# sanweiliti/RoHM

Hardware: AMD Instinct MI355X
Metric: denoised 145-frame clips/sec @1000 DDPM steps (higher is better)
Workload: dtype f32

## Files before the change

rohm_amd/csrc/common.h:

```cpp
#pragma once
#include <hip/hip_runtime.h>
#include <stdint.h>
#include <stdio.h>
#include <stdarg.h>
#include "../../include/rohm_hip.h"

typedef float f32x4 __attribute__((ext_vector_type(4)));
typedef float f32x2 __attribute__((ext_vector_type(2)));

namespace rohm {

void set_error(const char* fmt, ...);

#define ROHM_HIP_CHECK(expr)                                                             \
    do {                                                                                 \
        hipError_t _e = (expr);                                                          \
        if (_e != hipSuccess) {                                                          \
            rohm::set_error("%s failed: %s (%s:%d)", #expr, hipGetErrorString(_e), __FILE__, \
                            __LINE__);                                                   \
            return ROHM_ERR_HIP;                                                         \
        }                                                                                \
    } while (0)

#define ROHM_LAUNCH_CHECK()                                                              \
// ... 91 lines not shown
int exchange_layout_state(int device, const char** why);
int device_of_pointer(const void* ptr);

int launch_gemm(const GemmParams& p, int epi, hipStream_t s);

struct ChainParams {
    const float* ctx; float* h; float* y; float* ff; float* qkv;
    int M, D, F, tiles_m;
    const float *out_w, *out_b, *n1_w, *n1_b, *l1_w, *l1_b, *l2_w, *l2_b, *n2_w, *n2_b, *in_w, *in_b;
    float qscale, ln_eps;
    float* xln_stats; unsigned* xln_err; const unsigned* xln_pass; unsigned* xln_xcc; unsigned epoch;
    unsigned long long* flags;
    int fault;
};
struct StackLayerW { const float *out_w, *out_b, *n1_w, *n1_b, *l1_w, *l1_b, *l2_w, *l2_b, *n2_w, *n2_b, *in_w, *in_b; };
struct StackParams {
    float *h, *y, *ff, *qkv, *ctx;
    int M, D, F, tiles_m, L, n_head;
    float qscale, ln_eps;
    float* xln_stats; unsigned* xln_err; const unsigned* xln_pass; unsigned* xln_xcc; unsigned epoch;
    unsigned long long* flags;
    int fault;
    StackLayerW layer[8];
    const float* apack; int lda_pack; const float* w_embed; int ldw_embed; int k_embed;
    int S; const float* tab; const float* tab0; int ldtab, ldtab0, tab_by_row;
    const float* w_fold; int ldw_fold; const float* qtab; const float* qtab0;
    unsigned long long* timeline;
    int tail;
    const float* t_out_w; const float* t_out_b;
    float* t_x; const float* t_cond; const float* t_noise;
    float* t_x0; float* t_apack;
    float t_c1, t_c2, t_sigma;
    int t_traj, t_C, t_T, t_lda;
    unsigned* t_pass_ctr;
    unsigned pass_add;
};
constexpr int kStackTimelineLayers = 9, kStackTimelineStamps = 12;
int launch_encoder_stack(const StackParams& p, hipStream_t s);
int encoder_chain_parts(int M, int D, int F);
bool encoder_chain_pays(int B);
size_t encoder_chain_flag_bytes(int M);
int launch_encoder_chain(const ChainParams& p, hipStream_t s);
bool stream_is_capturing(hipStream_t s);
#ifdef __HIPCC__
__device__ __forceinline__ float wave_sum64(float v) {
    typedef unsigned rohm_u2 __attribute__((ext_vector_type(2)));
    rohm_u2 s = __builtin_amdgcn_permlane32_swap(__float_as_uint(v), __float_as_uint(v), false, false);
    v = __uint_as_float(s[0]) + __uint_as_float(s[1]);
    s = __builtin_amdgcn_permlane16_swap(__float_as_uint(v), __float_as_uint(v), false, false);
    v = __uint_as_float(s[0]) + __uint_as_float(s[1]);
// ... 31 lines not shown
```

rohm_amd/csrc/encoder_chain.hip:

```cpp
#include <type_traits>
#include "common.h"
#include "gemm_sched.h"
#include "attention_tile.h"

namespace rohm {

typedef float f32x16c __attribute__((ext_vector_type(16)));

namespace chain {

constexpr int BM = 144, BK = kGemmBK, NRB = BM / 16;
constexpr int A_UNITS = BM * 8, A_ITERS = (A_UNITS + 255) / 256;
constexpr int kMaxBN = 384;
constexpr int kZone = 2 * (BM + kMaxBN) * BK;
constexpr int kLdsFloats = kZone + 512 + 4 * BM * 2;
constexpr int kSc1 = 16;

struct PhaseArgs {
    const float* A; int lda;
    const float* W; int ldw;
    float* C; int ldc;
    int K;
    const float* bias;
    const float* R; int ldr;
// ... 42 lines not shown
            if ((it & 127) == 127 && __hip_atomic_load(err, __ATOMIC_RELAXED, __HIP_MEMORY_SCOPE_AGENT) != 0u) break;
            if (it > (1 << 19)) {
                __hip_atomic_store(err, 1u, __ATOMIC_RELAXED, __HIP_MEMORY_SCOPE_AGENT);
                break;
            }
        }
    }
    __syncthreads();
}

template <int BN, int EPI, bool PREF, bool SC1, bool REFETCH, bool HEAD = false, bool FOLD = false, typename AfterLoop>
__device__ __forceinline__ void gemm_phase(const PhaseArgs& p, float* smem, const int tid, AfterLoop&& after_loop,
                                           AtQFrags<2>* q_out = nullptr) {
    static_assert(EPI == EPI_BIAS_RES_LN || EPI == EPI_BIAS_GELU || EPI == EPI_QKV || EPI == EPI_EMBED, "chain phases: LN tail, GELU, QKV, embed");
    static_assert(!HEAD || (EPI == EPI_QKV && BN == 3 * AT_DH), "the head-aligned tile is one head's q | k | v");
    static_assert(!FOLD || (EPI == EPI_QKV && PREF && !SC1), "the folded in-projection: prefetched weights, A from an earlier launch");
    constexpr int WN = BN / 4;
    constexpr int NCB = WN / 16;
    constexpr int B_ITERS = BN * 8 / 256;
    constexpr int PIECES = A_ITERS + B_ITERS;
    constexpr int AUX = SC1 ? kSc1 : 0;

    float* As = smem;
    float* Bs = smem + 2 * BM * BK;
    float* lds_dummy = smem + kZone;
    float* const zone = lds_dummy + 512;
    float* const colrow = HEAD ? smem + 2 * AT_TILE : zone;
    static_assert(!HEAD || 2 * AT_TILE + 512 <= AT_LDS_FLOATS, "head-aligned tile: the bias row overruns the stack's LDS");

    const int lane = tid & 63;
    const int wave = tid >> 6;
// ... 346 lines not shown
#pragma unroll
                for (int q = 0; q < 4; ++q) v[q] = gelu_erf(v[q]);
            }
            if constexpr (EPI == EPI_QKV) {
                if (nb < p.qcols) {
#pragma unroll
                    for (int q = 0; q < 4; ++q) v[q] *= p.qscale;
                }
            }
            *reinterpret_cast<f32x4*>(p.C + (size_t)m * p.ldc + nb) = v;
        });
    }
}

template <int G>
__device__ __forceinline__ void head_tail_phase(const StackParams& p, const int g, const int tn, float* smem, const int tid) {
    constexpr int NC_OWN = 16 / G;
    constexpr int NW = NC_OWN * 16 + 16;
    constexpr int NRMAX = (G == 4) ? 9 : 5;
    constexpr int W_UNITS = NW * 8, W_ITERS = (W_UNITS + 255) / 256;
    constexpr int PIECES = A_ITERS + W_ITERS;
    constexpr int kBuf = (BM + NW) * BK;
    static_assert(3 * kBuf <= kZone, "head phase: staging buffers overrun the zone");
    float* lds_dummy = smem + kZone;
    const int lane = tid & 63, li = lane & 15, lg = lane >> 4;
    const int wave = __builtin_amdgcn_readfirstlane(tid >> 6);
    const int wave_u = wave * 64;
    const int D = p.D, m0 = g * BM;
    int c_loc, r0, nr, e;
    if constexpr (G == 4) { c_loc = wave; r0 = 0; nr = 9; e = tn * 4 + wave; }
    else { c_loc = wave >> 1; r0 = (wave & 1) ? 5 : 0; nr = (wave & 1) ? 4 : 5; e = (wave & 1) ? tn * 2 + (wave >> 1) : 99; }
// ... 33 lines not shown
            __builtin_amdgcn_global_load_lds((const __attribute__((address_space(1))) void*)(w_src[i] + k0),
                                             (__attribute__((address_space(3))) void*)dst, 16, 0, 0);
        }
    };

    f32x4 acc[NRMAX], acc_e = f32x4{0.f, 0.f, 0.f, 0.f};
#pragma unroll
    for (int r = 0; r < NRMAX; ++r) acc[r] = f32x4{0.f, 0.f, 0.f, 0.f};
    const int nk = D / BK;
    dma(0, 0);
    dma(1, BK);

    typedef float f32x4u __attribute__((ext_vector_type(4), aligned(4)));
    const int C = p.t_C, T = p.t_T, traj = p.t_traj, S = BM;
    float* const x = p.t_x;
    const float* const nzp = p.t_noise;
    const size_t row_own = ((size_t)g * C + traj + (tn * NC_OWN + c_loc) * 16 + li) * T;
    const size_t row_sh = ((size_t)g * C + traj + 256 + li) * T;
    f32x4 xt[NRMAX], nz[NRMAX], xt_e = f32x4{0.f, 0.f, 0.f, 0.f}, nz_e = f32x4{0.f, 0.f, 0.f, 0.f};
#pragma unroll
    for (int r = 0; r < NRMAX; ++r) {
        xt[r] = nz[r] = f32x4{0.f, 0.f, 0.f, 0.f};
        if (r < nr) {
            const size_t idx = row_own + (size_t)((r0 + r) * 16 + 4 * lg) - 1;
            xt[r] = *reinterpret_cast<const f32x4u*>(x + idx);
            if (nzp) nz[r] = *reinterpret_cast<const f32x4u*>(nzp + idx);
        }
    }
    if (has_e) {
        const size_t idx = row_sh + (size_t)(e * 16 + 4 * lg) - 1;
        xt_e = *reinterpret_cast<const f32x4u*>(x + idx);
// ... 47 lines not shown
            __syncthreads();
            __builtin_amdgcn_sched_barrier(0);
            if (kc + 2 < nk) dma(buf >= 1 ? buf - 1 : 2, (kc + 2) * BK);
            AT_WAIT_LGKM0();
            __builtin_amdgcn_sched_barrier(0);
            read_h(f0, nbuf, 0);
            __builtin_amdgcn_sched_barrier(0);
        } else {
            AT_WAIT_LGKM0();
        }
        mma_h(f1);
        __builtin_amdgcn_sched_barrier(0);
        buf = nbuf;
    }

    const float c1 = p.t_c1, c2 = p.t_c2, sg = p.t_sigma;
    float* const x0o = p.t_x0;
    float* const apk = p.t_apack;
    auto emit = [&](int rblk, size_t row, int ch, float bias, const f32x4& a, const f32x4& xv, const f32x4& nv) __attribute__((always_inline)) {
        const int tok0 = rblk * 16 + 4 * lg;
        f32x4 val, o;
#pragma unroll
        for (int v = 0; v < 4; ++v) {
            val[v] = a[v] + bias;
            o[v] = c1 * val[v] + c2 * xv[v];
            if (nzp) o[v] += sg * nv[v];
        }
        const size_t idx = row + (size_t)tok0 - 1;
        if (tok0 != 0) {
            if (x0o) *reinterpret_cast<f32x4u*>(x0o + idx) = val;
            *reinterpret_cast<f32x4u*>(x + idx) = o;
        } else {
#pragma unroll
// ... 65 lines not shown
    a.A = p.h; a.lda = p.D; a.W = p.in_w; a.ldw = p.D; a.C = p.qkv; a.ldc = 3 * p.D; a.K = p.D; a.bias = p.in_b; a.n0 = tn * BNQ;
    a.qcols = p.D; a.qscale = p.qscale;
    gemm_phase<BNQ, EPI_QKV, true, true, G == 8>(a, smem, tid, []() {});
}

template <int G>
__global__ __launch_bounds__(256) void encoder_stack_kernel(StackParams p) {
    using namespace chain;
    constexpr int BNL = 512 / G, BNF = 1024 / G, BNQ = 1536 / G;
    extern __shared__ __attribute__((aligned(16))) float smem[];
    const int tid0 = threadIdx.x;
    const int x = blockIdx.x % kNumXCD, j = blockIdx.x / kNumXCD;
    const int g = (j / G) * kNumXCD + x, tn = j % G;
    if (g >= p.tiles_m) return;
    const unsigned xcc1 = 1u + (unsigned)__builtin_amdgcn_s_getreg((3 << 11) | 20);
    const unsigned ep = p.epoch + 64u * (*p.xln_pass + p.pass_add);
    if (tid0 == 0) p.xln_xcc[g * 8 + tn] = xcc1;

    PhaseArgs a{};
    a.m0 = g * BM; a.err = p.xln_err; a.xcc1 = xcc1; a.tn = tn; a.tiles_n = G;
    a.row_stats = p.xln_stats + ((size_t)g * G * BM) * 4;
    a.eps = p.ln_eps; a.ln_dim = p.D;
    a.qcols = p.D; a.qscale = p.qscale;
    constexpr bool HEAD = G == 4;
    auto n0q = [&]() __attribute__((always_inline)) { return HEAD ? tn * AT_DH : tn * BNQ; };
    AtQFrags<2> qh;
    unsigned long long* const tl = p.timeline ? p.timeline + (size_t)blockIdx.x * kStackTimelineLayers * kStackTimelineStamps : nullptr;
    auto stamp = [&](int layer, int k) __attribute__((always_inline)) {
        if (tl != nullptr && threadIdx.x == 0) tl[layer * kStackTimelineStamps + k] = __builtin_amdgcn_s_memrealtime();
    };
    auto attend = [&](int l, int tid) __attribute__((always_inline)) {
        unsigned long long* const fl = p.flags + ((size_t)g * 9 + l) * 5 * 8;
        stamp(l, 0);
        if (l > 0) {
            if constexpr (HEAD) __syncthreads();
            else group_sync(fl, tn, G, ep, xcc1, p.xln_err, tid);
        }
        stamp(l, 1);
        if constexpr (HEAD)
            attention_item<4, 0, kSc1, 2, true>(p.qkv, p.ctx, p.n_head, g * p.n_head + tn, 0, AT_NB, smem, tid, &qh);
        else attention_item<4, 0, kSc1, 1>(p.qkv, p.ctx, p.n_head, g * p.n_head + (tn >> 1), (tn & 1) ? 5 : 0, (tn & 1) ? 4 : 5, smem, tid);
        stamp(l, 2);
        group_sync(fl + 8, tn, G, ep, xcc1, p.xln_err, tid);
        stamp(l, 3);
    };
    {
    int tid = tid0;
    asm volatile("" : "+v"(tid));
    const int wave_u = __builtin_amdgcn_readfirstlane(tid >> 6) * 64;
    unsigned long long* const fl = p.flags + ((size_t)g * 9 + 8) * 5 * 8;
    a.A = p.apack; a.lda = p.lda_pack; a.W = p.w_embed; a.ldw = p.ldw_embed; a.C = p.h; a.ldc = p.D; a.K = p.k_embed; a.n0 = tn * BNL;
    a.S = p.S; a.tab = p.tab; a.tab0 = p.tab0; a.ldtab = p.ldtab; a.ldtab0 = p.ldtab0; a.tab_by_row = p.tab_by_row;
    stamp(8, 0);
    const bool fold = p.w_fold != nullptr;
    gemm_phase<BNL, EPI_EMBED, false, false, G == 8>(a, smem, tid, [&]() {
        prefetch_w<BNQ, HEAD>(fold ? p.w_fold : p.layer[0].in_w, fold ? p.ldw_fold : p.D, n0q(), smem, tid, wave_u);
    });
    stamp(8, 1);
    a.C = p.qkv; a.ldc = 3 * p.D; a.n0 = n0q();
    if (fold) {
        asm volatile("s_waitcnt vmcnt(0)" ::: "memory");
        stamp(8, 2);
        a.W = p.w_fold; a.ldw = p.ldw_fold; a.tab = p.qtab; a.ldtab = 3 * p.D; a.tab0 = p.qtab0;
        gemm_phase<BNQ, EPI_QKV, true, false, G == 8, HEAD, true>(a, smem, tid, []() {}, &qh);
    } else {
        group_sync(fl, tn, G, ep, xcc1, p.xln_err, tid);
        stamp(8, 2);
        a.A = p.h; a.lda = p.D; a.W = p.layer[0].in_w; a.ldw = p.D; a.K = p.D; a.bias = p.layer[0].in_b;
        gemm_phase<BNQ, EPI_QKV, true, true, G == 8, HEAD>(a, smem, tid, []() {}, &qh);
    }
    stamp(8, 3);
    if constexpr (HEAD) __syncthreads();
    else group_sync(fl + 8, tn, G, ep, xcc1, p.xln_err, tid);
    stamp(8, 4);
    if constexpr (HEAD) attend(0, tid);
    }
#pragma unroll 1
    for (int l = 0; l < p.L; ++l) {
        int tid = tid0;
// ... 15 lines not shown
        gemm_phase<BNF, EPI_BIAS_GELU, true, true, G == 8>(a, smem, tid, [&]() { prefetch_w<BNL>(w.l2_w, p.F, tn * BNL, smem, tid, wave_u); });
        stamp(l, 6);
        group_sync(fl + 24, tn, G, ep, xcc1, p.xln_err, tid);
        stamp(l, 7);

        const bool more = l + 1 < p.L;
        a.A = p.ff; a.lda = p.F; a.W = w.l2_w; a.ldw = p.F; a.C = p.h; a.ldc = p.D; a.K = p.F; a.bias = w.l2_b;
        a.R = p.y; a.ldr = p.D; a.gamma = w.n2_w; a.beta = w.n2_b; a.n0 = tn * BNL; a.tag28 = (ep + 4u * l + 1u) & 0x0fffffffu;
        a.fault = (l == 0) ? ((p.fault >> 1) & 1) : 0;
        gemm_phase<BNL, EPI_BIAS_RES_LN, true, true, G == 8>(a, smem, tid, [&]() { if (more) prefetch_w<BNQ, HEAD>(p.layer[l + 1].in_w, p.D, n0q(), smem, tid, wave_u); });
        stamp(l, 8);
        if (!more) {
            if (p.tail) {
                group_sync(fl + 32, tn, G, ep, xcc1, p.xln_err, tid);
                stamp(l, 9);
                head_tail_phase<G>(p, g, tn, smem, tid);
                stamp(l, 10);
                if (p.t_pass_ctr != nullptr && blockIdx.x == 0 && threadIdx.x == 0) p.t_pass_ctr[1] = p.pass_add + 1u;
            }
            break;
        }
        group_sync(fl + 32, tn, G, ep, xcc1, p.xln_err, tid);
        stamp(l, 9);

        a.A = p.h; a.lda = p.D; a.W = p.layer[l + 1].in_w; a.ldw = p.D; a.C = p.qkv; a.ldc = 3 * p.D; a.K = p.D; a.bias = p.layer[l + 1].in_b;
        a.n0 = n0q();
        gemm_phase<BNQ, EPI_QKV, true, true, G == 8, HEAD>(a, smem, tid, []() {}, &qh);
        stamp(l, 10);
        if constexpr (HEAD) attend(l + 1, tid);
    }
}

int launch_encoder_stack(const StackParams& p, hipStream_t s) {
    const int G = encoder_chain_parts(p.M, p.D, p.F);
    ROHM_ARG_CHECK(G != 0 && p.n_head == 4 && p.L >= 1 && p.L <= 8, "encoder_stack: shape (M %d, D %d, F %d, %d heads, %d layers) has no stack form",
                   p.M, p.D, p.F, p.n_head, p.L);
    ROHM_ARG_CHECK(p.h && p.y && p.ff && p.qkv && p.ctx && p.xln_stats && p.xln_err && p.xln_pass && p.xln_xcc && p.flags, "encoder_stack: null operand");
    ROHM_ARG_CHECK(p.apack && p.w_embed && p.tab && p.tab0 && p.S == chain::BM && p.k_embed >= 2 * chain::BK && p.k_embed % chain::BK == 0 &&
                       p.lda_pack % 4 == 0 && p.ldw_embed % 4 == 0 && p.ldtab % 4 == 0 && p.ldtab0 % 4 == 0,
                   "encoder_stack: bad operands of the leading embed phase");
    StackParams q = p;
    q.tiles_m = p.M / chain::BM;
    const int groups8 = (q.tiles_m + kNumXCD - 1) / kNumXCD * kNumXCD;
    ROHM_ARG_CHECK(!p.w_fold || (p.qtab && p.qtab0 && p.ldw_fold % 4 == 0 && p.ldw_fold >= p.k_embed && p.tab_by_row),
                   "encoder_stack: bad operands of the folded in-projection");
    ROHM_ARG_CHECK(!p.tail || (p.D == 512 && p.t_out_w && p.t_out_b && p.t_x && p.t_cond && p.t_C - p.t_traj == 272 &&
                               p.t_T == chain::BM - 1 && p.t_traj > 0 && (!p.t_apack || p.t_lda >= p.t_C)),
                   "encoder_stack: the closing head / update / pack phase needs whole 144-token clips, d_model 512 and 272 predicted channels");
    constexpr int kFloats = AT_LDS_FLOATS > chain::kLdsFloats ? AT_LDS_FLOATS : chain::kLdsFloats;
    const size_t lds = (size_t)kFloats * sizeof(float);
    static bool attr_set[64][2] = {};
    int dev = 0;
    ROHM_HIP_CHECK(hipGetDevice(&dev));
    if (dev < 64 && !attr_set[dev][G == 8]) {
        if (G == 4) ROHM_HIP_CHECK(hipFuncSetAttribute(reinterpret_cast<const void*>(&encoder_stack_kernel<4>), hipFuncAttributeMaxDynamicSharedMemorySize, (int)lds));
        else ROHM_HIP_CHECK(hipFuncSetAttribute(reinterpret_cast<const void*>(&encoder_stack_kernel<8>), hipFuncAttributeMaxDynamicSharedMemorySize, (int)lds));
        attr_set[dev][G == 8] = true;
    }
    const double MM = (double)p.M, D = p.D, F = p.F, L = p.L;
    const double flops = L * (4.0 * 144.0 * 128.0 * MM * p.n_head + 2.0 * MM * (D * D + 2.0 * D * F)) + L * 2.0 * MM * 3.0 * D * D +
                         2.0 * MM * D * p.k_embed;
    const double bytes = 4.0 * (L * (MM * (3.0 * D + D + 4.0 * D + 2.0 * F + D) + D * D + 2.0 * D * F) + (L - 1.0) * (MM * 3.0 * D + 3.0 * D * D));
    const double tail_flops = p.tail ? 2.0 * MM * D * (p.t_C - p.t_traj) : 0.0;
    prof::Scope ps(p.tail ? "gemm_stack_tail" : "gemm_stack", flops + tail_flops, bytes, s);
    if (G == 4) hipLaunchKernelGGL(encoder_stack_kernel<4>, dim3(groups8 * 4), dim3(256), lds, s, q);
    else hipLaunchKernelGGL(encoder_stack_kernel<8>, dim3(groups8 * 8), dim3(256), lds, s, q);
    ROHM_LAUNCH_CHECK();
    return ROHM_OK;
}

int encoder_chain_parts(int M, int D, int F) {
    if (D != 512 || F != 1024 || M <= 0 || M % chain::BM != 0) return 0;
    const int tm = M / chain::BM;
    return tm >= 48 ? 4 : 8;
}

bool encoder_chain_pays(int B) {
    if (B <= 0) return false;
    if (B < 48) return B > 24 && B <= 32;
// ... 37 lines not shown
```

rohm_amd/csrc/posenet.hip:

```cpp
#include <stdlib.h>
#include <string.h>
#include <vector>
#include <atomic>
#include "common.h"
#include "planes.h"

namespace rohm {

constexpr int kMaxTok = 256;
constexpr int kLoopChunk = 1024;
constexpr float kF16WeightScale = 256.0f;

struct LayerW {
    float *in_w, *in_b, *out_w, *out_b, *l1_w, *l1_b, *l2_w, *l2_b, *n1_w, *n1_b, *n2_w, *n2_b;
    char *in_wp, *out_wp, *l1_wp, *l2_wp;
    char *l1_wpf, *in_wpf;
    float *l1_cf, *l1_df, *in_cf, *in_df;
};

}

struct rohm_posenet {
    int D, H, F, L, Cin, Cout, traj, device;
    int KP;
// ... 2 lines not shown
    int KX;
    float* w_embed_x;
    bool cond_hoist;
    float* w_fold;
    float* tokq;
    float* tab;
    float* pe;
    int pe_len;
    float *t_w0T, *t_b0, *t_w2T, *t_b2;
    float* tok_table;
    float *out_w, *out_b;
    bool ln_fused;
    bool head_sk;
    bool chain_any;
    bool stack_tail;
    int chain;
    bool ln_fused_env, head_sk_env;
    bool exch_allowed, exch_fallback;
    const char* exch_reason;
    unsigned salt;
    mutable int fault_left;
    unsigned long long* stack_timeline;
    int nplane;
    char* wplanes;
    bool pp_fold;
    float* foldvec;
    char* wplanes_fold;
    std::vector<rohm::LayerW> layers;
};

// ... 235 lines not shown
                        w.sk, 256 * sizeof(unsigned long long), false, s, w.chain_flags, encoder_chain_flag_bytes((int)M));
}
static inline unsigned* pass_counter(const Workspace& w) { return reinterpret_cast<unsigned*>(w.xln) + 2; }

static int check_shape(const rohm_posenet* p, int B, int T) {
    ROHM_ARG_CHECK(p != nullptr, "posenet: null handle");
    ROHM_ARG_CHECK(B > 0, "posenet: batch must be positive (got %d)", B);
    ROHM_ARG_CHECK(T + 1 <= kMaxTok && T + 1 <= p->pe_len, "posenet: sequence too long");
    return ROHM_OK;
}

static inline float qscale_of(const rohm_posenet* p) { return 1.0f / sqrtf((float)(p->D / p->H)); }

struct TailArgs {
    float* x; const float* cond; const float* noise; float* x0; float* apack_next;
    float c1, c2, sigma;
    unsigned* pass_ctr;
    int step;
};

struct EncoderPlan {
    bool planes;
    bool lnf;
    bool chained;
    bool stacked;
    bool tail;
};

static EncoderPlan plan_encoder(const rohm_posenet* p, int B, int S) {
    const int D = p->D, M = B * S;
    EncoderPlan e{};
    e.planes = p->nplane && S == 144 && D / p->H == 128;
    e.lnf = p->ln_fused && !e.planes && gemm_ln_supported(M, D, D) && gemm_ln_supported(M, D, p->F);
    e.chained = e.lnf && p->chain && encoder_chain_parts(M, D, p->F) != 0 && 4 * p->L + 2 <= 60 &&
                ((B >= 32 && encoder_chain_pays(B)) || p->chain_any);
    e.stacked = e.chained && p->chain == 2 && p->H == 4 && p->L <= 8 && S == 144 && D / p->H == 128;
    e.tail = e.stacked && p->stack_tail && D == 512 && p->Cout == 272;
    return e;
}

static int run_network(const rohm_posenet* p, const Workspace& w, const int64_t* t_dev, int64_t t_host,
                       const float* tok_pre, float* x0_out, int B, int T, hipStream_t s, bool cond_done = false,
                       const TailArgs* tail = nullptr, bool* tail_ran = nullptr, bool fold = false) {
    if (tail_ran) *tail_ran = false;
    const int S = T + 1, D = p->D, M = B * S;
    const float* tokq_row = nullptr;
    if (!tok_pre) {
        if (t_dev) {
            prof::Scope ps("gather_tokens", 0.0, 8.0 * D * B, s);
            hipLaunchKernelGGL(gather_tokens_kernel, dim3(B), dim3(256), 0, s, p->tok_table, p->pe_len, t_dev, w.tab0, D);
            ROHM_LAUNCH_CHECK();
        } else {
            int64_t t = t_host < 0 ? 0 : (t_host >= p->pe_len ? p->pe_len - 1 : t_host);
            tok_pre = p->tok_table + (size_t)t * D;
            if (p->tokq) tokq_row = p->tokq + (size_t)t * 3 * D;
        }
    }
    int rc;
    const EncoderPlan plan = plan_encoder(p, B, S);
    GemmParams ge{};
    ge.A = w.apack; ge.lda = p->KP; ge.W = p->w_embed; ge.ldw = p->KP; ge.C = w.h; ge.ldc = D;
// ... 63 lines not shown
            c.layer[l] = StackLayerW{lw.out_w, lw.out_b, lw.n1_w, lw.n1_b, lw.l1_w, lw.l1_b, lw.l2_w, lw.l2_b, lw.n2_w, lw.n2_b, lw.in_w, lw.in_b};
        }
        {
            GemmParams b{};
            b.M = M;
            gemm_ln_bind(b, w.xln);
            c.xln_stats = b.xln_stats; c.xln_err = b.xln_err; c.xln_pass = b.xln_pass; c.xln_xcc = b.xln_xcc;
        }
        c.epoch = p->salt;
        c.flags = reinterpret_cast<unsigned long long*>(w.chain_flags);
        if (p->fault_left > 0) { --p->fault_left; c.fault = 1; }
        c.timeline = p->stack_timeline;
        if (tail && plan.tail) {
            c.tail = 1;
            c.t_out_w = p->out_w; c.t_out_b = p->out_b;
            c.t_x = tail->x; c.t_cond = tail->cond; c.t_noise = tail->sigma == 0.f ? nullptr : tail->noise;
            c.t_x0 = tail->x0; c.t_apack = tail->apack_next;
            c.t_c1 = tail->c1; c.t_c2 = tail->c2; c.t_sigma = tail->sigma;
            c.t_traj = p->traj; c.t_C = p->Cin; c.t_T = T; c.t_lda = p->KP; c.t_pass_ctr = tail->pass_ctr;
            c.pass_add = (unsigned)tail->step;
        }
        if ((rc = launch_encoder_stack(c, s))) return rc;
        if (c.tail) {
            if (tail_ran) *tail_ran = true;
            return ROHM_OK;
        }
    }
    const float qscale = qscale_of(p);
    for (int l = 0; l < ((plan.chained && !plan.stacked) ? p->L : 0); ++l) {
        const LayerW& lw = p->layers[l];
        if (l == 0) {
            GemmParams g{};
            g.A = h; g.lda = D; g.W = lw.in_w; g.ldw = D; g.C = w.qkv; g.ldc = 3 * D; g.M = M; g.N = 3 * D; g.K = D;
            g.bias = lw.in_b; g.qcols = D; g.qscale = qscale;
            if ((rc = launch_gemm(g, EPI_QKV, s))) return rc;
// ... 93 lines not shown
    const int C = p->Cin;
    if (sigma == 0.f) noise = nullptr;
    dim3 grid((C + 31) / 32, (T + 31) / 32, B);
    prof::Scope ps("finish_pack", 0.0, 4.0 * (double)B * C * T * (noise ? 6 : 5), s);
    hipLaunchKernelGGL(finish_pack_kernel, grid, dim3(256), 0, s, x0, cond, x, noise, apack, c1, c2, sigma, p->traj, C, T, T + 1, p->KP, pass_ctr);
    ROHM_LAUNCH_CHECK();
    return ROHM_OK;
}

static int read_knobs(rohm_posenet* p) {
    auto off = [](const char* name) { const char* e = getenv(name); return e && e[0] == '0'; };
    p->ln_fused = !off("ROHM_POSENET_LN_FUSED");
    p->head_sk = !off("ROHM_POSENET_HEAD_SK");
    p->stack_tail = !off("ROHM_POSENET_STACK_TAIL");
    p->cond_hoist = !off("ROHM_POSENET_COND_HOIST");
    p->pp_fold = !off("ROHM_PP_LNFOLD");
    const char* any = getenv("ROHM_POSENET_CHAIN_ANY");
    p->chain_any = any && any[0] == '1';
    const char* chain = getenv("ROHM_POSENET_CHAIN");
    p->chain = 2;
    if (chain && chain[0] == '0') p->chain = 0;
    else if (chain && (!strcmp(chain, "layer") || !strcmp(chain, "1"))) p->chain = 1;
    else if (chain && *chain && strcmp(chain, "stack") && strcmp(chain, "2")) {
        set_error("posenet_create: ROHM_POSENET_CHAIN must be 0, layer or stack (got '%s')", chain);
        return ROHM_ERR_ARG;
    }
    const char* prec = getenv("ROHM_GEMM_PRECISION");
    p->nplane = 0;
    if (prec && !strcmp(prec, "bf16x6")) p->nplane = 3;
    else if (prec && !strcmp(prec, "bf16x3")) p->nplane = 2;
// ... 351 lines not shown
    if (hoist) {
        const int S = T + 1;
        ROHM_HIP_CHECK(hipMemset2DAsync(w.apack, (size_t)h->KP * sizeof(float), 0, (size_t)h->Cin * sizeof(float), (size_t)B * S, s));
        GemmParams g{};
        g.A = w.apack; g.lda = h->KP; g.W = h->w_embed; g.ldw = h->KP; g.C = w.econd; g.ldc = h->D;
        g.M = B * S; g.N = h->D; g.K = h->KP; g.S = S; g.tab = h->tab; g.tab0 = h->tok_table; g.ldtab = h->D; g.ldtab0 = 0;
        if ((rc = launch_gemm(g, EPI_EMBED, s))) return rc;
    }
    const bool fold = hoist && w.econdq && plan_encoder(h, B, T + 1).stacked;
    if (fold) {
        GemmParams g{};
        g.A = w.econd; g.lda = h->D; g.W = h->layers[0].in_w; g.ldw = h->D; g.C = w.econdq; g.ldc = 3 * h->D;
        g.M = B * (T + 1); g.N = 3 * h->D; g.K = h->D; g.bias = h->layers[0].in_b;
        if ((rc = launch_gemm(g, EPI_BIAS, s))) return rc;
    }
    for (int i = 0; i < n_steps; ++i) {
        prof::set_step(i);
        const float c1 = coef[3 * i], c2 = coef[3 * i + 1], sigma = coef[3 * i + 2];
        ROHM_ARG_CHECK(sigma == 0.f || noise, "posenet_sample_loop: noise is required when sigma != 0");
        if (x_in_last && i == n_steps - 1)
            ROHM_HIP_CHECK(hipMemcpyAsync(x_in_last, x, n * sizeof(float), hipMemcpyDeviceToDevice, s));
        if (i == 0 && (rc = launch_pack(h, x, w.apack, B, T, 0, s, pass_counter(w)))) return rc;
        float* x0 = (x0_last && i == n_steps - 1) ? x0_last : w.x0;
        const float* nz = noise ? noise + (size_t)i * n : nullptr;
        TailArgs tail{x, cond, nz, (x0_last && i == n_steps - 1) ? x0_last : nullptr, (i + 1 < n_steps) ? w.apack : nullptr,
                      c1, c2, sigma, pass_counter(w), i};
        bool tail_ran = false;
        if ((rc = run_network(h, w, nullptr, t_model[i], nullptr, x0, B, T, s, hoist, &tail, &tail_ran, fold))) return rc;
        if (tail_ran) continue;
        if (i + 1 < n_steps) {
            if ((rc = launch_finish_pack(h, x0, cond, x, nz, w.apack, c1, c2, sigma, B, T, pass_counter(w), s))) return rc;
        } else if ((rc = launch_finish(x0, cond, x, nz, x, c1, c2, sigma, h->traj, h->Cin, T, n, s))) {
            return rc;
        }
    }
    return ROHM_OK;
}

}
```

rohm_amd/stack_timeline.py:

```python
from __future__ import annotations

import numpy as np
import torch

from . import _lib
from ._lib import check, lib, ptr

LAYERS, STAMPS = 9, 12
TICK_US = 0.01
PEAK_F32_MFMA_TFLOPS = 157.3

SPANS = (('wait_qkv', 0, 1), ('attention', 1, 2), ('wait_ctx', 2, 3), ('out_proj_norm1', 3, 4), ('wait_y', 4, 5),
         ('linear1_gelu', 5, 6), ('wait_ff', 6, 7), ('linear2_norm2', 7, 8), ('wait_h', 8, 9), ('in_proj_next', 9, 10))
FRONT_SPANS = (('embed', 0, 1), ('wait_embed', 1, 2), ('in_proj_0', 2, 3), ('wait_qkv0', 3, 4))


def _flops_per_layer(B, D=512, F=1024, S=144, H=4):
    M = B * S
    return {'attention': 4.0 * S * S * (D // H) * H * B, 'out_proj_norm1': 2.0 * M * D * D, 'linear1_gelu': 2.0 * M * D * F,
            'linear2_norm2': 2.0 * M * F * D, 'in_proj_next': 2.0 * M * 3 * D * D}


def measure(net, B, T=143, reps=5, device='cuda:0', seed=0, steps_per_call=2):
    dev = torch.device(device)
    nat = net.native(dev)
    if not nat.exchange_mode & 32 or B < 32:
        return {'error': f'no encoder-stack launch at B = {B} on this handle (exchange_mode {nat.exchange_mode}: {nat.exchange_guard})'}
    G = 4 if B >= 48 else 8
    groups8 = (B + 7) // 8 * 8
    nbytes = lib().rohm_posenet_stack_timeline_bytes(B)
    buf = torch.zeros(nbytes // 8, dtype=torch.int64, device=dev)
    g = torch.Generator(device=dev).manual_seed(seed)
    x = torch.randn(B, 294, 1, T, device=dev, generator=g)
    cond = torch.randn(B, 294, 1, T, device=dev, generator=g)
    n = int(steps_per_call)
    noise = torch.randn(n, B, 294, 1, T, device=dev, generator=g)
    coef = np.asarray([[0.02, 0.98, 0.05]] * n, np.float32)
    net.sample_loop_native(x, cond, [500 - k for k in range(n)], coef, noise)
# ... 9 lines not shown
            wall.append(e0.elapsed_time(e1) * 1e3 / n)
            recs.append(buf.cpu().numpy().reshape(-1, LAYERS, STAMPS)[:groups8 * G].astype(np.float64) * TICK_US)
    finally:
        check(lib().rohm_posenet_set_stack_timeline(nat.handle, None, 0, 0), 'rohm_posenet_set_stack_timeline')
    net.check_exchange()
    blocks = np.arange(groups8 * G)
    clip = (blocks // 8 // G) * 8 + blocks % 8
    valid = clip < B
    fl = _flops_per_layer(B)
    out = {'batch': B, 'parts_per_clip': G, 'workgroups': int(valid.sum()), 'launches_stamped': reps,
           'step_wall_us_by_events': float(np.median(wall)),
           'clock': 's_memrealtime (100 MHz wall clock), lane 0 of every workgroup; spans are means over workgroups, summed over the 8 layers'}
    spans, launch, finish = {}, [], []
    for Tm in recs:
        Tm = Tm[valid]
        front = Tm[:, 8, 0].min() > 0
        tail = Tm[:, 7, 10].min() > 0
        t0 = Tm[:, 8, 0].min() if front else Tm[:, 0, 0].min()
        last = Tm[:, 7, 10] if tail else Tm[:, 7, 8]
        t1 = last.max()
        launch.append(t1 - t0)
        for name, a, b in SPANS:
            tot = 0.0
            for l in range(8):
                if (name == 'wait_qkv' and l == 0) or (name == 'in_proj_next' and l == 7) or (name == 'wait_h' and l == 7 and not tail):
                    continue
                tot += float((Tm[:, l, b] - Tm[:, l, a]).mean())
            spans.setdefault(name, []).append(tot)
        if tail:
            spans.setdefault('head_update_pack', []).append(float((Tm[:, 7, 10] - Tm[:, 7, 9]).mean()))
# ... 34 lines not shown
    cors = [float(np.corrcoef(F[a], F[b])[0, 1]) for a in range(len(F)) for b in range(a + 1, len(F))]
    out['finish_skew_analysis'] = {
        'per_xcd_mean_us_behind_first': [round(float(v), 2) for v in per_xcd.mean(axis=0)],
        'per_xcd_std_over_launches_us': [round(float(v), 2) for v in per_xcd.std(axis=0)],
        'mean_over_workgroups_us_behind_first': round(float(F.mean()), 2),
        'correlation_of_workgroup_lateness_between_launches': round(float(np.mean(cors)), 3) if cors else None,
        'max_of_mean_lateness_us': round(float(mean_wg.max()), 2),
        'note': 'lateness = a workgroup\'s last stamp minus the launch\'s first finisher; correlation near 1 = the same workgroups are late in '
                'every launch (systematic: placement, XCD), near 0 = random'}
    waits = sum(v['us_per_launch'] for k, v in out['phases'].items() if k.startswith('wait_'))
    out['meetings_us_per_launch'] = round(waits, 2)
    out['meetings_share_of_launch'] = round(waits / span, 4)
    return out


def text(rec):
    if 'error' in rec:
        return rec['error']
    lines = [f"encoder_stack_kernel<{rec['parts_per_clip']}> at B = {rec['batch']}: {rec['workgroups']} workgroups, {rec['launches_stamped']} launches stamped; "
             f"launch span {rec['launch_span_us']:.1f} us (denoising step by events: {rec['step_wall_us_by_events']:.1f} us)",
             f"{'phase':<18}{'us / launch':>12}{'share':>9}{'TFLOP/s':>10}{'of 157.3':>10}"]
    for name, v in rec['phases'].items():
        lines.append(f"{name:<18}{v['us_per_launch']:>12.1f}{v['share_of_launch']:>9.3f}"
                     f"{v.get('tflops', float('nan')):>10.1f}{v.get('frac_of_fp32_mfma_peak', float('nan')):>10.3f}")
    a = rec['attention_in_stack']
    lines.append(f"meetings (all waits): {rec['meetings_us_per_launch']:.1f} us = {rec['meetings_share_of_launch']:.3f} of the launch")
    fa = rec.get('finish_skew_analysis')
    if fa:
        lines.append(f"finish skew: mean lateness {fa['mean_over_workgroups_us_behind_first']} us, per XCD {fa['per_xcd_mean_us_behind_first']} "
                     f"(std over launches {fa['per_xcd_std_over_launches_us']}), lateness correlation between launches "
# ... 5 lines not shown
```

Before: 23.80.

## Run multiple denoising steps inside one persistent encoder-stack launch

Adds a per-launch step table so the persistent encoder stack kernel loops over up to 16 DDPM steps by default, each with its own coefficients, timestep token row and noise slice. A group sync between steps replaces the kernel launch boundary. The intent is to remove per-step launch and host overhead along with the pipeline drain and refill between launches. In exchange the kernel arguments grow to nearly 4 KB, the embed phase now prefetches the packed A from the same launch, and the epoch and pass counters advance per step, which the sync logic must handle correctly.

```diff
diff --git a/rohm_amd/csrc/common.h b/rohm_amd/csrc/common.h
--- a/rohm_amd/csrc/common.h
+++ b/rohm_amd/csrc/common.h
@@ -129,6 +129,12 @@
     int fault;
 };
 struct StackLayerW { const float *out_w, *out_b, *n1_w, *n1_b, *l1_w, *l1_b, *l2_w, *l2_b, *n2_w, *n2_b, *in_w, *in_b; };
+struct StackStep {
+    int t_flags;
+    float c1, c2, sigma;
+};
+constexpr int kStepX0 = 1 << 16, kStepPack = 1 << 17, kStepNoise = 1 << 18;
+constexpr int kStackMaxSteps = 64;
 struct StackParams {
     float *h, *y, *ff, *qkv, *ctx;
     int M, D, F, tiles_m, L, n_head;
@@ -145,10 +151,11 @@
     const float* t_out_w; const float* t_out_b;
     float* t_x; const float* t_cond; const float* t_noise;
     float* t_x0; float* t_apack;
-    float t_c1, t_c2, t_sigma;
     int t_traj, t_C, t_T, t_lda;
     unsigned* t_pass_ctr;
     unsigned pass_add;
+    int n_steps, tab0_step, qtab0_step;
+    StackStep step[kStackMaxSteps];
 };
 constexpr int kStackTimelineLayers = 9, kStackTimelineStamps = 12;
 int launch_encoder_stack(const StackParams& p, hipStream_t s);
diff --git a/rohm_amd/csrc/encoder_chain.hip b/rohm_amd/csrc/encoder_chain.hip
--- a/rohm_amd/csrc/encoder_chain.hip
+++ b/rohm_amd/csrc/encoder_chain.hip
@@ -80,7 +80,7 @@
                                            AtQFrags<2>* q_out = nullptr) {
     static_assert(EPI == EPI_BIAS_RES_LN || EPI == EPI_BIAS_GELU || EPI == EPI_QKV || EPI == EPI_EMBED, "chain phases: LN tail, GELU, QKV, embed");
     static_assert(!HEAD || (EPI == EPI_QKV && BN == 3 * AT_DH), "the head-aligned tile is one head's q | k | v");
-    static_assert(!FOLD || (EPI == EPI_QKV && PREF && !SC1), "the folded in-projection: prefetched weights, A from an earlier launch");
+    static_assert(!FOLD || (EPI == EPI_QKV && PREF), "the folded in-projection: prefetched weights");
     constexpr int WN = BN / 4;
     constexpr int NCB = WN / 16;
     constexpr int B_ITERS = BN * 8 / 256;
@@ -457,7 +457,8 @@
 }
 
 template <int G>
-__device__ __forceinline__ void head_tail_phase(const StackParams& p, const int g, const int tn, float* smem, const int tid) {
+__device__ __forceinline__ void head_tail_phase(const StackParams& p, const StackStep st, const float* const nzp, const int g, const int tn,
+                                                float* smem, const int tid) {
     constexpr int NC_OWN = 16 / G;
     constexpr int NW = NC_OWN * 16 + 16;
     constexpr int NRMAX = (G == 4) ? 9 : 5;
@@ -521,7 +522,6 @@
     typedef float f32x4u __attribute__((ext_vector_type(4), aligned(4)));
     const int C = p.t_C, T = p.t_T, traj = p.t_traj, S = BM;
     float* const x = p.t_x;
-    const float* const nzp = p.t_noise;
     const size_t row_own = ((size_t)g * C + traj + (tn * NC_OWN + c_loc) * 16 + li) * T;
     const size_t row_sh = ((size_t)g * C + traj + 256 + li) * T;
     f32x4 xt[NRMAX], nz[NRMAX], xt_e = f32x4{0.f, 0.f, 0.f, 0.f}, nz_e = f32x4{0.f, 0.f, 0.f, 0.f};
@@ -599,9 +599,9 @@
         buf = nbuf;
     }
 
-    const float c1 = p.t_c1, c2 = p.t_c2, sg = p.t_sigma;
-    float* const x0o = p.t_x0;
-    float* const apk = p.t_apack;
+    const float c1 = st.c1, c2 = st.c2, sg = st.sigma;
+    float* const x0o = (st.t_flags & kStepX0) ? p.t_x0 : nullptr;
+    float* const apk = (st.t_flags & kStepPack) ? p.t_apack : nullptr;
     auto emit = [&](int rblk, size_t row, int ch, float bias, const f32x4& a, const f32x4& xv, const f32x4& nv) __attribute__((always_inline)) {
         const int tok0 = rblk * 16 + 4 * lg;
         f32x4 val, o;
@@ -697,7 +697,8 @@
     const int g = (j / G) * kNumXCD + x, tn = j % G;
     if (g >= p.tiles_m) return;
     const unsigned xcc1 = 1u + (unsigned)__builtin_amdgcn_s_getreg((3 << 11) | 20);
-    const unsigned ep = p.epoch + 64u * (*p.xln_pass + p.pass_add);
+    const unsigned pass0 = *p.xln_pass + p.pass_add;
+    unsigned ep = p.epoch + 64u * pass0;
     if (tid0 == 0) p.xln_xcc[g * 8 + tn] = xcc1;
 
     PhaseArgs a{};
@@ -727,16 +728,22 @@
         group_sync(fl + 8, tn, G, ep, xcc1, p.xln_err, tid);
         stamp(l, 3);
     };
+    const int n_steps = p.tail ? p.n_steps : 1;
+#pragma unroll 1
+    for (int step = 0; step < n_steps; ++step) {
+    const StackStep st = p.step[step];
+    const int t_row = st.t_flags & 0xffff;
+    ep = p.epoch + 64u * (pass0 + (unsigned)step);
     {
     int tid = tid0;
     asm volatile("" : "+v"(tid));
     const int wave_u = __builtin_amdgcn_readfirstlane(tid >> 6) * 64;
     unsigned long long* const fl = p.flags + ((size_t)g * 9 + 8) * 5 * 8;
     a.A = p.apack; a.lda = p.lda_pack; a.W = p.w_embed; a.ldw = p.ldw_embed; a.C = p.h; a.ldc = p.D; a.K = p.k_embed; a.n0 = tn * BNL;
-    a.S = p.S; a.tab = p.tab; a.tab0 = p.tab0; a.ldtab = p.ldtab; a.ldtab0 = p.ldtab0; a.tab_by_row = p.tab_by_row;
+    a.S = p.S; a.tab = p.tab; a.tab0 = p.tab0 + (size_t)p.tab0_step * t_row; a.ldtab = p.ldtab; a.ldtab0 = p.ldtab0; a.tab_by_row = p.tab_by_row;
     stamp(8, 0);
     const bool fold = p.w_fold != nullptr;
-    gemm_phase<BNL, EPI_EMBED, false, false, G == 8>(a, smem, tid, [&]() {
+    gemm_phase<BNL, EPI_EMBED, false, true, G == 8>(a, smem, tid, [&]() {
         prefetch_w<BNQ, HEAD>(fold ? p.w_fold : p.layer[0].in_w, fold ? p.ldw_fold : p.D, n0q(), smem, tid, wave_u);
     });
     stamp(8, 1);
@@ -744,8 +751,8 @@
     if (fold) {
         asm volatile("s_waitcnt vmcnt(0)" ::: "memory");
         stamp(8, 2);
-        a.W = p.w_fold; a.ldw = p.ldw_fold; a.tab = p.qtab; a.ldtab = 3 * p.D; a.tab0 = p.qtab0;
-        gemm_phase<BNQ, EPI_QKV, true, false, G == 8, HEAD, true>(a, smem, tid, []() {}, &qh);
+        a.W = p.w_fold; a.ldw = p.ldw_fold; a.tab = p.qtab; a.ldtab = 3 * p.D; a.tab0 = p.qtab0 + (size_t)p.qtab0_step * t_row;
+        gemm_phase<BNQ, EPI_QKV, true, true, G == 8, HEAD, true>(a, smem, tid, []() {}, &qh);
     } else {
         group_sync(fl, tn, G, ep, xcc1, p.xln_err, tid);
         stamp(8, 2);
@@ -791,9 +798,14 @@
             if (p.tail) {
                 group_sync(fl + 32, tn, G, ep, xcc1, p.xln_err, tid);
                 stamp(l, 9);
-                head_tail_phase<G>(p, g, tn, smem, tid);
+                const float* const nzp = (st.t_flags & kStepNoise) ? p.t_noise + (size_t)step * ((size_t)p.tiles_m * p.t_C * p.t_T) : nullptr;
+                head_tail_phase<G>(p, st, nzp, g, tn, smem, tid);
                 stamp(l, 10);
-                if (p.t_pass_ctr != nullptr && blockIdx.x == 0 && threadIdx.x == 0) p.t_pass_ctr[1] = p.pass_add + 1u;
+                if (step + 1 < n_steps) {
+                    group_sync(p.flags + ((size_t)g * 9 + 8) * 5 * 8 + 16, tn, G, ep, xcc1, p.xln_err, tid);
+                } else if (p.t_pass_ctr != nullptr && blockIdx.x == 0 && threadIdx.x == 0) {
+                    p.t_pass_ctr[1] = p.pass_add + (unsigned)n_steps;
+                }
             }
             break;
         }
@@ -805,6 +817,7 @@
         gemm_phase<BNQ, EPI_QKV, true, true, G == 8, HEAD>(a, smem, tid, []() {}, &qh);
         stamp(l, 10);
         if constexpr (HEAD) attend(l + 1, tid);
+    }
     }
 }
 
@@ -824,6 +837,17 @@
     ROHM_ARG_CHECK(!p.tail || (p.D == 512 && p.t_out_w && p.t_out_b && p.t_x && p.t_cond && p.t_C - p.t_traj == 272 &&
                                p.t_T == chain::BM - 1 && p.t_traj > 0 && (!p.t_apack || p.t_lda >= p.t_C)),
                    "encoder_stack: the closing head / update / pack phase needs whole 144-token clips, d_model 512 and 272 predicted channels");
+    static_assert(sizeof(StackParams) < 4096, "encoder_stack: the step table must leave the kernel arguments under 4 KB");
+    const int n_steps = p.tail ? p.n_steps : 1;
+    ROHM_ARG_CHECK(n_steps >= 1 && n_steps <= kStackMaxSteps && (n_steps == 1 || (p.t_apack && !p.timeline && !p.fault)),
+                   "encoder_stack: %d steps in one launch (1 .. %d; more than one needs the pack, no timeline, no injected fault)", p.n_steps,
+                   kStackMaxSteps);
+    for (int i = 0; i < n_steps && p.tail; ++i) {
+        const int f = p.step[i].t_flags;
+        ROHM_ARG_CHECK((i + 1 == n_steps || (f & kStepPack)) && (!(f & kStepNoise) || p.t_noise) && (!(f & kStepX0) || p.t_x0) &&
+                           (!(f & kStepPack) || p.t_apack),
+                       "encoder_stack: step %d of the launch lacks an operand its flags ask for", i);
+    }
     constexpr int kFloats = AT_LDS_FLOATS > chain::kLdsFloats ? AT_LDS_FLOATS : chain::kLdsFloats;
     const size_t lds = (size_t)kFloats * sizeof(float);
     static bool attr_set[64][2] = {};
@@ -839,7 +863,7 @@
                          2.0 * MM * D * p.k_embed;
     const double bytes = 4.0 * (L * (MM * (3.0 * D + D + 4.0 * D + 2.0 * F + D) + D * D + 2.0 * D * F) + (L - 1.0) * (MM * 3.0 * D + 3.0 * D * D));
     const double tail_flops = p.tail ? 2.0 * MM * D * (p.t_C - p.t_traj) : 0.0;
-    prof::Scope ps(p.tail ? "gemm_stack_tail" : "gemm_stack", flops + tail_flops, bytes, s);
+    prof::Scope ps(p.tail ? "gemm_stack_tail" : "gemm_stack", (flops + tail_flops) * n_steps, bytes * n_steps, s);
     if (G == 4) hipLaunchKernelGGL(encoder_stack_kernel<4>, dim3(groups8 * 4), dim3(256), lds, s, q);
     else hipLaunchKernelGGL(encoder_stack_kernel<8>, dim3(groups8 * 8), dim3(256), lds, s, q);
     ROHM_LAUNCH_CHECK();
diff --git a/rohm_amd/csrc/posenet.hip b/rohm_amd/csrc/posenet.hip
--- a/rohm_amd/csrc/posenet.hip
+++ b/rohm_amd/csrc/posenet.hip
@@ -8,6 +8,7 @@
 namespace rohm {
 
 constexpr int kMaxTok = 256;
+constexpr int kStackStepsDefault = 16;
 constexpr int kLoopChunk = 1024;
 constexpr float kF16WeightScale = 256.0f;
 
@@ -40,6 +41,7 @@
     bool head_sk;
     bool chain_any;
     bool stack_tail;
+    int stack_steps;
     int chain;
     bool ln_fused_env, head_sk_env;
     bool exch_allowed, exch_fallback;
@@ -305,9 +307,9 @@
 
 struct TailArgs {
     float* x; const float* cond; const float* noise; float* x0; float* apack_next;
-    float c1, c2, sigma;
     unsigned* pass_ctr;
     int step;
+    int n_steps; const StackStep* steps;
 };
 
 struct EncoderPlan {
@@ -336,6 +338,7 @@
     if (tail_ran) *tail_ran = false;
     const int S = T + 1, D = p->D, M = B * S;
     const float* tokq_row = nullptr;
+    const bool t_from_table = !tok_pre && !t_dev;
     if (!tok_pre) {
         if (t_dev) {
             prof::Scope ps("gather_tokens", 0.0, 8.0 * D * B, s);
@@ -429,11 +432,19 @@
         if (tail && plan.tail) {
             c.tail = 1;
             c.t_out_w = p->out_w; c.t_out_b = p->out_b;
-            c.t_x = tail->x; c.t_cond = tail->cond; c.t_noise = tail->sigma == 0.f ? nullptr : tail->noise;
+            c.t_x = tail->x; c.t_cond = tail->cond; c.t_noise = tail->noise;
             c.t_x0 = tail->x0; c.t_apack = tail->apack_next;
-            c.t_c1 = tail->c1; c.t_c2 = tail->c2; c.t_sigma = tail->sigma;
             c.t_traj = p->traj; c.t_C = p->Cin; c.t_T = T; c.t_lda = p->KP; c.t_pass_ctr = tail->pass_ctr;
             c.pass_add = (unsigned)tail->step;
+            ROHM_ARG_CHECK(tail->n_steps >= 1 && tail->n_steps <= kStackMaxSteps && (tail->n_steps == 1 || t_from_table) &&
+                               (!t_from_table || p->pe_len <= 65536),
+                           "posenet: %d steps in one stack launch", tail->n_steps);
+            c.n_steps = tail->n_steps;
+            for (int k = 0; k < tail->n_steps; ++k) c.step[k] = tail->steps[k];
+            if (t_from_table) {
+                c.tab0 = p->tok_table; c.tab0_step = D;
+                if (c.w_fold) { c.qtab0 = p->tokq; c.qtab0_step = 3 * D; }
+            }
         }
         if ((rc = launch_encoder_stack(c, s))) return rc;
         if (c.tail) {
@@ -557,6 +568,16 @@
     p->head_sk = !off("ROHM_POSENET_HEAD_SK");
     p->stack_tail = !off("ROHM_POSENET_STACK_TAIL");
     p->cond_hoist = !off("ROHM_POSENET_COND_HOIST");
+    p->stack_steps = kStackStepsDefault;
+    if (const char* e = getenv("ROHM_POSENET_STACK_STEPS"); e && *e) {
+        char* end = nullptr;
+        const long v = strtol(e, &end, 10);
+        if (*end != 0 || v < 1 || v > kStackMaxSteps) {
+            set_error("posenet_create: ROHM_POSENET_STACK_STEPS must be 1 .. %d (got '%s')", kStackMaxSteps, e);
+            return ROHM_ERR_ARG;
+        }
+        p->stack_steps = (int)v;
+    }
     p->pp_fold = !off("ROHM_PP_LNFOLD");
     const char* any = getenv("ROHM_POSENET_CHAIN_ANY");
     p->chain_any = any && any[0] == '1';
@@ -938,20 +959,44 @@
         g.M = B * (T + 1); g.N = 3 * h->D; g.K = h->D; g.bias = h->layers[0].in_b;
         if ((rc = launch_gemm(g, EPI_BIAS, s))) return rc;
     }
-    for (int i = 0; i < n_steps; ++i) {
+    for (int i = 0; i < 3 * n_steps; i += 3)
+        ROHM_ARG_CHECK(coef[i + 2] == 0.f || noise, "posenet_sample_loop: noise is required when sigma != 0");
+    const int group_max = plan_encoder(h, B, T + 1).tail ? h->stack_steps : 1;
+    auto step_of = [&](int i) {
+        const int64_t t = t_model[i] < 0 ? 0 : (t_model[i] >= h->pe_len ? h->pe_len - 1 : t_model[i]);
+        StackStep st{(int)t, coef[3 * i], coef[3 * i + 1], coef[3 * i + 2]};
+        if (x0_last && i == n_steps - 1) st.t_flags |= kStepX0;
+        if (i + 1 < n_steps) st.t_flags |= kStepPack;
+        if (st.sigma != 0.f) st.t_flags |= kStepNoise;
+        return st;
+    };
+    for (int i = 0, n_group = 1; i < n_steps; i += n_group) {
         prof::set_step(i);
-        const float c1 = coef[3 * i], c2 = coef[3 * i + 1], sigma = coef[3 * i + 2];
-        ROHM_ARG_CHECK(sigma == 0.f || noise, "posenet_sample_loop: noise is required when sigma != 0");
+        StackStep steps[kStackMaxSteps];
+        steps[0] = step_of(i);
+        n_group = 1;
+        if (group_max > 1 && !prof::g_active && !h->stack_timeline && h->fault_left <= 0) {
+            for (int j = i + 1; j < n_steps && n_group < group_max; ++j) {
+                if (x_in_last && j == n_steps - 1) break;
+                prof::set_step(j);
+                if (prof::g_active) break;
+                steps[n_group++] = step_of(j);
+            }
+            prof::set_step(i);
+        }
+        const float c1 = steps[0].c1, c2 = steps[0].c2, sigma = steps[0].sigma;
         if (x_in_last && i == n_steps - 1)
             ROHM_HIP_CHECK(hipMemcpyAsync(x_in_last, x, n * sizeof(float), hipMemcpyDeviceToDevice, s));
         if (i == 0 && (rc = launch_pack(h, x, w.apack, B, T, 0, s, pass_counter(w)))) return rc;
         float* x0 = (x0_last && i == n_steps - 1) ? x0_last : w.x0;
         const float* nz = noise ? noise + (size_t)i * n : nullptr;
-        TailArgs tail{x, cond, nz, (x0_last && i == n_steps - 1) ? x0_last : nullptr, (i + 1 < n_steps) ? w.apack : nullptr,
-                      c1, c2, sigma, pass_counter(w), i};
+        const int i_end = i + n_group;
+        TailArgs tail{x, cond, nz, (x0_last && i_end == n_steps) ? x0_last : nullptr, (i + 1 < n_steps) ? w.apack : nullptr,
+                      pass_counter(w), i, n_group, steps};
         bool tail_ran = false;
         if ((rc = run_network(h, w, nullptr, t_model[i], nullptr, x0, B, T, s, hoist, &tail, &tail_ran, fold))) return rc;
         if (tail_ran) continue;
+        ROHM_ARG_CHECK(n_group == 1, "posenet_sample_loop: grouped steps need the stack's closing phase");
         if (i + 1 < n_steps) {
             if ((rc = launch_finish_pack(h, x0, cond, x, nz, w.apack, c1, c2, sigma, B, T, pass_counter(w), s))) return rc;
         } else if ((rc = launch_finish(x0, cond, x, nz, x, c1, c2, sigma, h->traj, h->Cin, T, n, s))) {
diff --git a/rohm_amd/stack_timeline.py b/rohm_amd/stack_timeline.py
--- a/rohm_amd/stack_timeline.py
+++ b/rohm_amd/stack_timeline.py
@@ -21,7 +21,7 @@
             'linear2_norm2': 2.0 * M * F * D, 'in_proj_next': 2.0 * M * 3 * D * D}
 
 
-def measure(net, B, T=143, reps=5, device='cuda:0', seed=0, steps_per_call=2):
+def measure(net, B, T=143, reps=5, device='cuda:0', seed=0, steps_per_call=2, stamps=None):
     dev = torch.device(device)
     nat = net.native(dev)
     if not nat.exchange_mode & 32 or B < 32:
@@ -61,6 +61,8 @@
     spans, launch, finish = {}, [], []
     for Tm in recs:
         Tm = Tm[valid]
+        if stamps is not None:
+            stamps.append(Tm.copy())
         front = Tm[:, 8, 0].min() > 0
         tail = Tm[:, 7, 10].min() > 0
         t0 = Tm[:, 8, 0].min() if front else Tm[:, 0, 0].min()
@@ -125,6 +127,12 @@
     return out
 
 
+def stamps_xcd(B):
+    G = 4 if B >= 48 else 8
+    blocks = np.arange((B + 7) // 8 * 8 * G)
+    return (blocks % 8)[(blocks // 8 // G) * 8 + blocks % 8 < B]
+
+
 def text(rec):
     if 'error' in rec:
         return rec['error']
```

After: 23.97, median of 6. Within noise of the previous version (+0.7%).
